# mjq11302010044/TATT

Measured on AMD Instinct MI355X. Metric: LR images/s (train fwd+bwd+clip+Adam) at 16x64->32x128, higher is better.
Workload: dtype fp32 (split-bf16 MFMA operands in conv3 / conv3-wgrad / conv9 / tokgemm / gru-wgrad / query-GRU recurrence and dW_hh / TP-layer backward)

## Files before the change

include/tatt_hip.h:

```cpp
#ifndef TATT_HIP_H
#define TATT_HIP_H

#ifdef __cplusplus
extern "C" {
#endif

typedef struct ihipStream_t* hipStream_t;


int tatt_gemm(const float* A, long sam, long sak, const float* A2, long sa2m, long sa2k, int K1,
              const float* B, long sbk, long sbn, const float* bias, float* C, long scm, long scn,
              int M, int N, int K, int Z, long bsA, long bsA2, long bsB, long bsC, long bsBias,
              float alpha, float beta, int act, int splitk, float* ws, float* rowsum, hipStream_t st);

int tatt_conv2d_fwd(const float* x, long xsn, long xsh, long xsw, long xsc, const float* wpacked,
                    const float* bias, float* y, long ldy, int Bn, int H, int W, int Cin, int Cout,
                    int KH, int KW, int act, float beta, int splitk, float* ws, hipStream_t st);

int tatt_conv2d_fwd_partials(const float* x, long xsn, long xsh, long xsw, long xsc, const float* wpacked, int Bn, int H,
                             int W, int Cin, int Cout, int KH, int KW, int splitk, float* ws, int* splits, hipStream_t st);

int tatt_conv2d_wgrad(const float* x, long xsn, long xsh, long xsw, long xsc, const float* dy,
                      long lddy, float* dw_oihw, int Bn, int H, int W, int Cin, int Cout, int KH,
                      int KW, float beta, int splitk, float* ws, hipStream_t st);
// ... 64 lines not shown
                         const float* beta, float* mean, float* rstd, float* running_mean, float* running_var, float* scale,
                         float* shift, hipStream_t st);
int tatt_bn_rstd(const float* var, float* rstd, int C, float eps, hipStream_t st);
int tatt_bn_apply(const float* X, long ldx, float* Y, long ldy, int M, int C, const float* mean,
                  const float* rstd, const float* gamma, const float* beta, int act, hipStream_t st);
int tatt_bn_bwd(const float* X, long ldx, const float* dY, long lddy, float* dX, long lddx, int M, int C,
                const float* mean, const float* rstd, const float* gamma, const float* beta, int act,
                int training, float* dgamma, float* dbeta, float* sums, double* ws, hipStream_t st);
int tatt_bn_bwd_groups(int M);
int tatt_bn_bwd_partials(const float* X, long ldx, const float* dY, long lddy, int M, int C, const float* mean,
                         const float* rstd, const float* gamma, const float* beta, int act, double* part, hipStream_t st);
int tatt_bn_bwd_finish(const double* part, int G, int C, int M, const float* mean, const float* rstd, const float* gamma,
                       float* dgamma, float* dbeta, float* coef, hipStream_t st);
int tatt_bn_bwd_affine(const float* X, const float* dU, float* dX, int M, int C, const float* coef, hipStream_t st);

int tatt_ln_fwd(const float* A, const float* Bres, float* Y, float* stats, int M, int C,
                const float* gamma, const float* beta, float eps, int mode, float pdrop,
                const unsigned long long* seed, unsigned site, hipStream_t st);
int tatt_ln_bwd(const float* A, const float* Bres, const float* dY, const float* stats, float* dX, float* dB, int M,
                int C, const float* gamma, float* dgamma, float* dbeta, float* part, double* ws, float eps, int mode,
                float pdrop, const unsigned long long* seed, unsigned site, hipStream_t st);


int tatt_prelu_fwd(const float* x, float* y, const float* alpha, long n, hipStream_t st);
int tatt_prelu_bwd(const float* x, const float* dy, float* dx, const float* alpha, long n, float* part,
                   hipStream_t st);
int tatt_act_fwd(const float* x, float* y, long n, int act, hipStream_t st);
int tatt_act_bwd(const float* ref, const float* dy, float* dx, long n, int act, int from_output,
                 hipStream_t st);
int tatt_axpby(const float* a, const float* b, float* y, float alpha, float beta, long n, hipStream_t st);
int tatt_add_n(const float* const* srcs, int n, float* y, long numel, hipStream_t st);
int tatt_add_rowbcast(const float* a, const float* b, float* y, long rows, int C, long period,
                      hipStream_t st);
int tatt_pixel_shuffle_fwd(const float* in, float* out, int B, int H, int W, int C, int act,
                           hipStream_t st);
int tatt_pixel_shuffle_bwd(const float* in, const float* dout, float* din, int B, int H, int W, int C,
                           int act, hipStream_t st);
int tatt_maxpool_fwd(const float* in, float* out, int B, int H, int W, int C, int kh, int kw, int sh, int sw,
                     int ph, int pw, hipStream_t st);
int tatt_maxpool_bwd(const float* in, const float* dout, float* din, int B, int H, int W, int C, int kh,
                     int kw, int sh, int sw, int ph, int pw, hipStream_t st);
int tatt_dropout(const float* x, float* y, long n, float p, const unsigned long long* seed, unsigned site,
                 hipStream_t st);
int tatt_bump_seed(unsigned long long* seed, unsigned long long* snap, hipStream_t st);
int tatt_stamp(unsigned long long* out, hipStream_t st);
int tatt_copy4d(const float* src, float* dst, int n0, int n1, int n2, int n3, long s0, long s1, long s2,
                long s3, long d0, long d1, long d2, long d3, float beta, hipStream_t st);


int tatt_l2norm(const float* g, long n, float* out, double* ws, hipStream_t st);
int tatt_adam_step(float* p, const float* g, float* m, float* v, long n, float lr, float b1, float b2,
                   float eps, const float* gnorm, float max_norm, float gscale, const long long* step,
                   hipStream_t st);


int tatt_gru32_fwd(const float* gi, const float* whh_f, const float* bhh_f, const float* whh_r,
                   const float* bhh_r, float* out, float* gates, int nseq, int T, int s_in, long stride_hi,
                   long stride_lo, long stride_t, hipStream_t st);
int tatt_gru32_bwd(const float* gates, const float* out, const float* dout, const float* whh_f,
                   const float* whh_r, float* dgi, float* dgh, float* hprev, int nseq, int T, int s_in,
                   long stride_hi, long stride_lo, long stride_t, hipStream_t st);

int tatt_gru32_fwd2(const float* gi, const float* whh_f, const float* bhh_f, const float* whh_r,
                    const float* bhh_r, float* out, float* gates, int nseq, int T, int s_in, long stride_hi,
                    long stride_lo, long stride_t, hipStream_t st);
int tatt_gru32_bwd2(const float* gates, const float* out, const float* dout, const float* whh_f,
                    const float* whh_r, float* dgi, float* dgh, float* hprev, float* frag, int nseq, int T, int s_in,
                    long stride_hi, long stride_lo, long stride_t, hipStream_t st);
int tatt_gru_wgrad_frag(const float* frag, const float* x, const float* xb, float* ws1, float* ws2, int nseq, int T,
                        int s_in, long stride_hi, long stride_lo, long stride_t, int G, hipStream_t st);
int tatt_gru_wgrad_frag_in(const float* frag, const float* x, const float* xb, float* ws1, float* ws2, int nseq, int T,
                           int s_in, long stride_hi, long stride_lo, long stride_t, int G, const float* in_mean,
                           const float* in_rstd, const float* in_gamma, const float* in_beta, const float* in_add,
                           hipStream_t st);

int tatt_qgru_bwd_fused(const float* dgh_cur0, const float* dgh_cur1, const float* whhT0, const float* whhT1,
                        const float* dhseq_next0, const float* dhseq_next1, const float* gsave_next0,
                        const float* gsave_next1, const float* hprev_next0, const float* hprev_next1,
                        float* dhcarry0, float* dhcarry1, float* dgi_acc0, float* dgi_acc1, float* dgh_next0,
                        float* dgh_next1, int Wb, int HID, hipStream_t st);

int tatt_gru_compose(const float* wih_f, const float* wih_r, const float* bih_f, const float* bih_r,
                     const float* Wc, const float* bc, float* Wp, float* bp, int K, hipStream_t st);
int tatt_gru_compose_batch(const float* const* ptrs, const int* Ks, int n, hipStream_t st);
int tatt_gru_tail(const float* dWp, const float* dbp, const float* Wc, const float* bc, const float* wih_f,
                  const float* wih_r, float* dwih_f, float* dwih_r, float* dWc, float* dbc, int K,
                  const float* dWhh, float* dwhh_f, float* dwhh_r, hipStream_t st);

int tatt_gru_tail_c(const float* dWp, const float* dbp, const float* Wc, const float* bc, const float* wih_f,
                    const float* wih_r, float* dwih_f, float* dwih_r, float* dWc, float* dbc, int K,
                    const float* dWhh_c, float* dwhh_f, float* dwhh_r, hipStream_t st);

int tatt_qgru_fwd_step(const float* gi0, const float* gi1, const float* whh0, const float* whh1,
                       const float* bhh0, const float* bhh1, const float* hprev0, const float* hprev1,
                       float* hnew0, float* hnew1, float* gsave0, float* gsave1, int Wb, int HID,
                       hipStream_t st);
int tatt_qgru_bwd_gates(const float* dhseq0, const float* dhseq1, const float* gsave0, const float* gsave1,
                        const float* hprev0, const float* hprev1, float* dhcarry0, float* dhcarry1,
                        float* dgi_acc0, float* dgi_acc1, float* dgh0, float* dgh1, int Wb, int HID, int first,
                        hipStream_t st);
int tatt_qgru_bwd_mm(const float* dgh0, const float* dgh1, const float* whhT0, const float* whhT1,
                     float* dhcarry0, float* dhcarry1, int Wb, int HID, hipStream_t st);

int tatt_qgru_bwd_chain(float* dgh0, float* dgh1, const float* whhT0, const float* whhT1, const float* dhseq0,
                        const float* dhseq1, const float* gsave0, const float* gsave1, const float* hbuf0,
                        const float* hbuf1, float* dhcarry0, float* dhcarry1, float* dgi_acc0, float* dgi_acc1,
// ... 270 lines not shown
```

tatt_amd/csrc/elementwise.hip:

```cpp
#include "common.h"

#define EW_GRID(total) dim3(cdiv((total), 256)), dim3(256)

__global__ void prelu_fwd_kernel(const float* __restrict__ x, float* __restrict__ y, const float* __restrict__ a,
                                 long n) {
    long i = (long)blockIdx.x * blockDim.x + threadIdx.x;
    if (i >= n) return;
    float v = x[i];
    y[i] = v >= 0.f ? v : a[0] * v;
}
TATT_API int tatt_prelu_fwd(const float* x, float* y, const float* alpha, long n, hipStream_t st) {
    hipLaunchKernelGGL(prelu_fwd_kernel, EW_GRID(n), 0, st, x, y, alpha, n);
    return LAUNCH_CHECK();
}
__global__ void prelu_bwd_kernel(const float* __restrict__ x, const float* __restrict__ dy, float* __restrict__ dx,
                                 const float* __restrict__ a, long n, float* __restrict__ part) {
    __shared__ double sh[4];
    long i = (long)blockIdx.x * blockDim.x + threadIdx.x;
    double s = 0.0;
    if (i < n) {
        float v = x[i], g = dy[i];
        dx[i] = v >= 0.f ? g : a[0] * g;
        if (v < 0.f) s = (double)g * (double)v;
    }
// ... 319 lines not shown
    s = wave_sum_d(s);
    if ((threadIdx.x & 63) == 0) sh[threadIdx.x >> 6] = s;
    __syncthreads();
    if (threadIdx.x == 0) out[0] = (float)sqrt((sh[0] + sh[1]) + (sh[2] + sh[3]));
}
TATT_API int tatt_l2norm(const float* g, long n, float* out, double* ws, hipStream_t st) {
    int G = (int)((n + 255) / 256);
    if (G > 1024) G = 1024;
    if (G < 1) G = 1;
    hipLaunchKernelGGL(sumsq_stage1, dim3(G), dim3(256), 0, st, g, n, ws);
    hipLaunchKernelGGL(sumsq_stage2, dim3(1), dim3(256), 0, st, ws, G, out);
    return LAUNCH_CHECK();
}
__device__ __forceinline__ void adam_one(float& p, float g, float& m, float& v, float coef, float b1, float b2, float a1, float rs2,
                                         float eps) {
    const float gi = g * coef;
    const float mi = b1 * m + (1.f - b1) * gi;
    const float vi = b2 * v + (1.f - b2) * gi * gi;
    m = mi; v = vi;
    p -= a1 * mi / (sqrtf(vi) * rs2 + eps);
}
__global__ void adam_kernel(float* __restrict__ p, const float* __restrict__ g, float* __restrict__ m,
                            float* __restrict__ v, long n, float lr, float b1, float b2, float eps,
                            const float* __restrict__ gnorm, float max_norm, float gscale,
                            const long long* __restrict__ step) {
    const long i = (long)blockIdx.x * blockDim.x + threadIdx.x;
    const long n4 = n >> 2;
    if (i > n4) return;
    const double t = (double)step[0];
    const float bc1 = (float)(1.0 - pow((double)b1, t)), bc2 = (float)(1.0 - pow((double)b2, t));
    float coef = gscale;
    if (max_norm > 0.f) { float c = max_norm / (gnorm[0] * gscale + 1e-6f); coef *= c < 1.f ? c : 1.f; }
    const float a1 = lr / bc1, rs2 = 1.f / sqrtf(bc2);
    if (i < n4) {
        float4 pp = ((float4*)p)[i], mm = ((float4*)m)[i], vv = ((float4*)v)[i];
        const float4 gg = ((const float4*)g)[i];
        adam_one(pp.x, gg.x, mm.x, vv.x, coef, b1, b2, a1, rs2, eps);
        adam_one(pp.y, gg.y, mm.y, vv.y, coef, b1, b2, a1, rs2, eps);
        adam_one(pp.z, gg.z, mm.z, vv.z, coef, b1, b2, a1, rs2, eps);
        adam_one(pp.w, gg.w, mm.w, vv.w, coef, b1, b2, a1, rs2, eps);
        ((float4*)p)[i] = pp; ((float4*)m)[i] = mm; ((float4*)v)[i] = vv;
    } else {
        for (long k = n4 << 2; k < n; ++k) adam_one(p[k], g[k], m[k], v[k], coef, b1, b2, a1, rs2, eps);
    }
}
TATT_API int tatt_adam_step(float* p, const float* g, float* m, float* v, long n, float lr, float b1, float b2,
                            float eps, const float* gnorm, float max_norm, float gscale, const long long* step,
                            hipStream_t st) {
    if (((uintptr_t)p | (uintptr_t)g | (uintptr_t)m | (uintptr_t)v) & 15) return 1001;
    hipLaunchKernelGGL(adam_kernel, EW_GRID((n >> 2) + 1), 0, st, p, g, m, v, n, lr, b1, b2, eps, gnorm, max_norm, gscale, step);
    return LAUNCH_CHECK();
}

#include <mutex>
static std::mutex g_sticky_mu;
static unsigned* g_sticky[64] = {};
unsigned* tatt_sticky_ptr() {
    int dev = 0;
    if (hipGetDevice(&dev) != hipSuccess || dev < 0 || dev >= 64) return nullptr;
    std::lock_guard<std::mutex> lk(g_sticky_mu);
    return g_sticky[dev];
}
TATT_API int tatt_set_sticky(unsigned* word) {
    int dev = 0;
    if (hipGetDevice(&dev) != hipSuccess || dev < 0 || dev >= 64) return 1;
    std::lock_guard<std::mutex> lk(g_sticky_mu);
    g_sticky[dev] = word;
    return 0;
}
__global__ void sync_guard_kernel(const unsigned* word) {
    if (__hip_atomic_load(word, __ATOMIC_RELAXED, __HIP_MEMORY_SCOPE_AGENT) != 0u) __builtin_trap();
}
TATT_API int tatt_sync_guard(hipStream_t st) {
    unsigned* w = tatt_sticky_ptr();
    if (!w) return 0;
    hipLaunchKernelGGL(sync_guard_kernel, dim3(1), dim3(1), 0, st, w);
    return LAUNCH_CHECK();
}

__global__ __launch_bounds__(512) void cu_holder_kernel(long ticks, unsigned* sink, int lds_words) {
    extern __shared__ unsigned hold_lds[];
    for (int i = threadIdx.x; i < lds_words; i += 512) hold_lds[i] = i;
    __syncthreads();
    const long t0 = wall_clock64();
    unsigned acc = 0;
    while (wall_clock64() - t0 < ticks) {
        acc += lds_words ? hold_lds[(threadIdx.x + acc) % lds_words] : 1u;
        __builtin_amdgcn_s_sleep(8);
    }
    if (acc == 0xffffffffu && sink) sink[0] = acc;
}
TATT_API int tatt_cu_holder(int groups, long ticks, int lds_bytes, unsigned* sink, hipStream_t st) {
    if (groups < 1 || groups > 1024 || ticks < 0 || ticks > 100000000L || lds_bytes < 0 || lds_bytes > 65536) return 1;
    hipLaunchKernelGGL(cu_holder_kernel, dim3(groups), dim3(512), lds_bytes, st, ticks, sink, lds_bytes / 4);
    return LAUNCH_CHECK();
}

#define GG_MAX 112
struct GGEntry { const float* src; long off; int n; int block0; };
struct GGTable { GGEntry e[GG_MAX]; float* dst; int n; };
__global__ __launch_bounds__(256) void gather_grads_kernel(GGTable t) {
    int k = 0;
    while (k + 1 < t.n && (int)blockIdx.x >= t.e[k + 1].block0) ++k;
    const GGEntry& e = t.e[k];
    const long i = ((long)((int)blockIdx.x - e.block0) * 256 + threadIdx.x) * 4;
    if (i >= e.n) return;
// ... 42 lines not shown
```

tatt_amd/csrc/gemm.hip:

```cpp
#include "common.h"
#include <mutex>
#include <unordered_map>
#include <stdlib.h>

#define BM 64
#define BN 64
#define KC 16
#define LDT 65

struct GemmP {
    const float* A; const float* A2; const float* B; const float* bias; float* C;
    int M, N, K, K1;
    long sam, sak, sa2m, sa2k, sbk, sbn, scm, scn;
    long bsA, bsA2, bsB, bsC, bsBias;
    float alpha, beta;
    int act;
    int splitk, chunks_per_split;
    float* partial;
    float* rowsum;
    int H, W, Cin, KH, KW, pad, HW, Wshift, HWshift, Cshift;
    long xsn, xsh, xsw, xsc;
};

__device__ __forceinline__ void decode_pixel(const GemmP& p, int pix, int& n, int& h, int& w) {
// ... 882 lines not shown
    if (mode >= 12) {
        if (idx < TOEPLITZ9_WORDS) out[idx] = toeplitz9_sb(w, idx, mode);
        return;
    }
    if (mode >= 10) {
        if (idx < Cout * Cin * 9) out[idx] = repack_sb(w, idx, Cout, Cin, mode);
        return;
    }
    if (mode >= 8) {
        if (idx < TOEPLITZ9_WORDS) out[idx] = toeplitz9(w, idx, mode);
        return;
    }
    int total = Cout * Cin * KH * KW;
    if (idx >= total) return;
    int T = KH * KW;
    if (mode == 0) {
        int co = idx % Cout; int r = idx / Cout; int ci = r % Cin; int tap = r / Cin;
        out[idx] = w[((long)co * Cin + ci) * T + tap];
    } else if (mode == 1) {
        int ci = idx % Cin; int r = idx / Cin; int co = r % Cout; int tap = r / Cout;
        out[idx] = w[((long)co * Cin + ci) * T + (T - 1 - tap)];
    } else if (mode == 2) {
        int ci = idx % Cin; int r = idx / Cin; int co = r % Cout; int tap = r / Cout;
        out[idx] = w[((long)co * Cin + ci) * T + tap];
    } else if (mode == 3) {
        int co = idx % Cout; int r = idx / Cout; int ci = r % Cin; int tap = r / Cin;
        out[idx] = w[((long)co * Cin + ci) * T + (T - 1 - tap)];
    } else {
        const int u = idx & 3, lane = (idx >> 2) & 63;
        const int q6 = (idx >> 8) % 36, blk = idx / (36 * 256);
        const int tap6 = q6 >> 2, g6 = q6 & 3;
        const int o6 = blk * 16 + (lane & 15), i6 = 16 * g6 + 4 * (lane >> 4) + u;
        if (mode == 6) out[idx] = w[((long)o6 * Cin + i6) * T + tap6];
        else out[idx] = w[((long)i6 * Cin + o6) * T + (T - 1 - tap6)];
    }
}
TATT_API int tatt_repack_words(int Cout, int Cin, int KH, int KW, int mode) {
    if (mode == 4 || mode == 5 || mode < 0 || mode > 15) return -1;
    return (int)repack_total(Cout, Cin, KH, KW, mode);
}
TATT_API int tatt_repack_conv_weight(const float* w_oihw, float* out, int Cout, int Cin, int KH, int KW,
                                     int mode, hipStream_t st) {
    const bool fwd9 = mode == 8 || mode == 12, dgrad9 = mode == 9 || mode == 13;
    if ((fwd9 || dgrad9) && !(KH == 9 && KW == 9 && ((fwd9 && Cout == 4 && Cin == 64) || (dgrad9 && Cout == 64 && Cin == 4)))) return 1;
    if ((mode == 10 || mode == 11 || mode == 14 || mode == 15) && !(KH == 3 && KW == 3 && Cout % 64 == 0 && Cin % 64 == 0)) return 1;
    if (mode == 4 || mode == 5 || mode < 0 || mode > 15) return 1;
    long total = repack_total(Cout, Cin, KH, KW, mode);
    hipLaunchKernelGGL(repack_weight_kernel, dim3(cdiv(total, 256)), dim3(256), 0, st, w_oihw, out, Cout, Cin,
                       KH, KW, mode);
    return LAUNCH_CHECK();
}

#define REPACK_MAX 96
struct RepackEntry { const float* w; float* out; int Cout, Cin, KH, KW, mode, block0; };
struct RepackTable { RepackEntry e[REPACK_MAX]; int n; };
__global__ void repack_batch_kernel(RepackTable t) {
    int k = 0;
    while (k + 1 < t.n && (int)blockIdx.x >= t.e[k + 1].block0) ++k;
    const RepackEntry& e = t.e[k];
    const int idx = ((int)blockIdx.x - e.block0) * blockDim.x + threadIdx.x;
    if (e.mode >= 14) {
        if (idx < e.Cout * e.Cin * 9) e.out[idx] = repack_sb32(e.w, idx, e.Cout, e.Cin, e.mode);
        return;
    }
    if (e.mode >= 12) {
        if (idx < TOEPLITZ9_WORDS) e.out[idx] = toeplitz9_sb(e.w, idx, e.mode);
        return;
    }
    if (e.mode >= 10) {
        if (idx < e.Cout * e.Cin * 9) e.out[idx] = repack_sb(e.w, idx, e.Cout, e.Cin, e.mode);
        return;
    }
    if (e.mode >= 8) {
        if (idx < TOEPLITZ9_WORDS) e.out[idx] = toeplitz9(e.w, idx, e.mode);
        return;
    }
    const int total = e.Cout * e.Cin * e.KH * e.KW;
    if (idx >= total) return;
    const int T = e.KH * e.KW, Cout = e.Cout, Cin = e.Cin;
    const float* w = e.w;
    float v;
    if (e.mode == 0) { int co = idx % Cout; int r = idx / Cout; int ci = r % Cin; int tap = r / Cin; v = w[((long)co * Cin + ci) * T + tap]; }
    else if (e.mode == 1) { int ci = idx % Cin; int r = idx / Cin; int co = r % Cout; int tap = r / Cout; v = w[((long)co * Cin + ci) * T + (T - 1 - tap)]; }
    else if (e.mode == 2) { int ci = idx % Cin; int r = idx / Cin; int co = r % Cout; int tap = r / Cout; v = w[((long)co * Cin + ci) * T + tap]; }
    else if (e.mode == 3) { int co = idx % Cout; int r = idx / Cout; int ci = r % Cin; int tap = r / Cin; v = w[((long)co * Cin + ci) * T + (T - 1 - tap)]; }
    else {
        const int u = idx & 3, lane = (idx >> 2) & 63;
        const int q6 = (idx >> 8) % 36, blk = idx / (36 * 256);
        const int tap6 = q6 >> 2, g6 = q6 & 3;
        const int o6 = blk * 16 + (lane & 15), i6 = 16 * g6 + 4 * (lane >> 4) + u;
        v = e.mode == 6 ? w[((long)o6 * Cin + i6) * T + tap6] : w[((long)i6 * Cin + o6) * T + (T - 1 - tap6)];
    }
    e.out[idx] = v;
}
TATT_API int tatt_repack_conv_weight_batch(const float* const* ws, float* const* outs, const int* dims, int n, hipStream_t st) {
    if (n <= 0) return 0;
    for (int base = 0; base < n; base += REPACK_MAX) {
        RepackTable t;
        t.n = n - base < REPACK_MAX ? n - base : REPACK_MAX;
        int blocks = 0;
        for (int k = 0; k < t.n; ++k) {
            const int* d = dims + (long)(base + k) * 5;
            t.e[k] = {ws[base + k], outs[base + k], d[0], d[1], d[2], d[3], d[4], blocks};
            blocks += cdiv(repack_total(d[0], d[1], d[2], d[3], d[4]), 256);
        }
        hipLaunchKernelGGL(repack_batch_kernel, dim3(blocks), dim3(256), 0, st, t);
    }
    return LAUNCH_CHECK();
}

TATT_API int tatt_splitk_reduce(const float* partial, float* C, int M, int N, int S, int remap_cin, int remap_taps,
                                float beta, float* vec, int vec_len, hipStream_t st) {
    ReduceArgs a = {partial, C, nullptr, vec, (long)N, 1L, 0L, 0L, M, N, S, 1, 1.f, beta, (int)ACT_NONE, remap_cin, remap_taps, 0,
                    vec ? vec_len : 0};
    return reduce_submit(a, st);
}
```

tatt_amd/train.py:

```python
from __future__ import annotations

import os
from typing import Optional

import torch

from . import functional as Fh
from . import ops
from .dp import FlatParams, GradCuts, broadcast_model, rank_dropout_seed


def image_loss(sr, hr, weights=(1.0, 1e-4)):
    return Fh.ImageLossFn.apply(sr, hr, float(weights[0]), float(weights[1]), None)


def image_loss_mean(sr, hr, weights=(1.0, 1e-4), scale=100.0):
    return Fh.ImageLossFn.apply(sr, hr, float(weights[0]), float(weights[1]), float(scale))


def semantic_loss(pred, gt):
    return Fh.SemanticLossFn.apply(pred, gt.detach())


_CTC_ROW_OFFS = {}
# ... 205 lines not shown
STUDENT_FORK = False
TEACHER_AHEAD = True


class TssimRecipe:

    def __init__(self, rotate_train=5.0, seed=0, off_range=0.2):
        import numpy as np
        self.rotate_train, self.off_range = float(rotate_train), off_range
        self.rng = np.random.RandomState(seed)
        self.theta_pos = self.theta_neg = None
        self.last = None

    def draw(self, B):
        import math
        arcs = torch.tensor((self.rng.rand(B) * self.rotate_train * 2 - self.rotate_train) / 180.0 * math.pi).float()
        offs = torch.tensor(self.rng.rand(B)).float()
        return arcs, offs

    def new_step(self, x, arcs=None, offs=None):
        from .losses import rotation_theta
        B, _, H, W = x.shape
        if arcs is None:
            arcs, offs = self.draw(B)
        self.last = (arcs, offs)
        pos, neg = rotation_theta(arcs, offs, H, W, self.off_range), rotation_theta(-arcs, offs, H, W, self.off_range)
        if self.theta_pos is None:
            self.theta_pos, self.theta_neg = pos.to(x.device), neg.to(x.device)
        else:
            self.theta_pos.copy_(pos)
            self.theta_neg.copy_(neg)

    def loss(self, model, x, tp, hr):
        from .losses import TRI_SSIM
        rot = Fh.AffineSampleFn.apply
        with torch.no_grad():
            x_rot, hr_rot = rot(x, self.theta_pos), rot(hr, self.theta_pos)
            x_ret = rot(x_rot, self.theta_neg)
        fwd = (lambda im: model(im, tp)) if tp is not None else model
        fwd_ret = (lambda im: model(im, reuse_prior=True)) if (tp is None and hasattr(model, "tpg")) else fwd
        if hasattr(model, "begin_teacher"):
            model.begin_teacher(hr_rot)
        out = fwd(x_rot)
        sr = out[0] if isinstance(out, tuple) else out
        extra = model.extra_loss(hr_rot) if hasattr(model, "extra_loss") else None
        out = fwd_ret(x_ret)
        sr_ret = out[0] if isinstance(out, tuple) else out
        l_img = image_loss_mean(sr, hr_rot, scale=100.0)
        l_tssim = (1.0 - TRI_SSIM()(rot(sr_ret, self.theta_pos), sr, hr_rot)) * 10.0
        loss = l_img + l_tssim
        return loss if extra is None else loss + extra


class HipStepKernels:

    def l2norm(self, g, out, ws):
        ops.call("tatt_l2norm", ops.P(g), g.numel(), ops.P(out), ops.P(ws), ops.stream())

    def adam(self, p, g, m, v, lr, b1, b2, eps, gnorm, max_norm, gscale, step):
        ops.call("tatt_adam_step", ops.P(p), ops.P(g), ops.P(m), ops.P(v), p.numel(), lr, b1, b2, eps, ops.P(gnorm), max_norm,
                 gscale, ops.P(step), ops.stream())

    def inc(self, counter):
        ops.inc_i64(counter)

    def guard(self):
        ops.call("tatt_sync_guard", ops.stream())

    def after_update(self, device):
        ops.PACKED.refresh(device)


def _default_loss(sr, hr):
    return image_loss_mean(sr, hr, scale=100.0)


class Trainer:

    def __init__(self, model, lr=1e-3, betas=(0.5, 0.999), eps=1e-8, clip=0.25, use_graph=False, warmup_eager=2,
                 process_group=None, broadcast_init=True, defer_param_grads=True, side_stream=True, kernels=None, loss_fn=None,
                 dropout_seed=None, recipe=None):
        self.model = model
        self.lr, self.betas, self.eps, self.clip = lr, betas, eps, clip
        self.pg = process_group
        self.dp = process_group is not None
        self.world = torch.distributed.get_world_size(process_group) if self.dp else 1
        self.rank = torch.distributed.get_rank(process_group) if self.dp else 0
        self.kernels = kernels if kernels is not None else HipStepKernels()
        self.loss_fn = loss_fn if loss_fn is not None else _default_loss
        self.recipe = recipe
        self.profile_collectives = False
        self._coll_events = []
        self._group_events = []
        dev = next(model.parameters()).device
        self.dev = dev
        self.cuda = dev.type == "cuda"
        self.defer = bool(defer_param_grads)
        self.two_lanes = self.defer and bool(side_stream) and self.cuda
        staged = (self.dp or self.defer) and hasattr(model, "grad_buckets") and hasattr(model, "set_grad_cuts")
        buckets = None
        if hasattr(model, "grad_buckets"):
            import inspect
            takes_dp = "dp" in inspect.signature(model.grad_buckets).parameters
            buckets = model.grad_buckets(dp=self.dp) if takes_dp else model.grad_buckets()
        if buckets is not None and not staged:
            buckets = [("all", [p for _, ps in buckets for p in ps])]
        self.flat = FlatParams(model, buckets)
        self.stages = self.flat.bucket_names
        self._due = {id(p): k for k, (_, ps) in enumerate(buckets or []) for p in ps}
        self._immediate = frozenset(id(p) for p in model.immediate_grad_params()) if hasattr(model, "immediate_grad_params") else frozenset()
        self.cuts = GradCuts() if staged and len(self.stages) > 1 else None
        self.params = self.flat.params
        self.n = self.flat.n
        self.flat_p, self.flat_g = self.flat.p, self.flat.g
        self.flat_m = torch.zeros(self.n, device=dev)
        self.flat_v = torch.zeros(self.n, device=dev)
        groups = model.clip_groups(clip) if hasattr(model, "clip_groups") else [(self.params, clip)]
        self.groups = [self.flat.span(ps) + (float(c),) for ps, c in groups]
        assert sorted(self.groups)[0][0] == 0 and sum(e - s for s, e, _ in self.groups) == self.n
        if self.dp and broadcast_init:
# ... 50 lines not shown
                    extra = self.model.extra_loss(hr) if hasattr(self.model, "extra_loss") else None
                    if extra is not None:
                        loss = loss + extra
                if self._one is None or self._one.device != loss.device or self._one.dtype != loss.dtype:
                    self._one = torch.ones_like(loss)
                loss.backward(self._one)
                self.last_loss = loss.detach()
            else:
                self.cuts.run(self.stages[k])
        finally:
            Fh.SIDE.enabled = False
            Fh.SIDE.side_stream = None
            Fh.FWD_FORK.enabled = Fh.FWD_FORK_B.enabled = False
            if k == 0 and self.cuts is not None:
                self.model.set_grad_cuts(None)
        if k == len(self.stages) - 1 and hasattr(self.model, "block"):
            self.model.block = None

    def _side_lane(self, k):
        Fh.SIDE.flush(None if k == len(self.stages) - 1 else k)
        self.flat.gather_grads(k)

    def _pass(self, k, x=None, tp=None, hr=None):
        nst = len(self.stages)
        main = torch.cuda.current_stream(self.dev) if self.cuda else None
        merge_last = self._merge_last
        if merge_last and k == nst:
            return
        name = self.stages[k] if k < nst and isinstance(self.stages[k], str) else str(k)
        Fh.stamp("pass %s: start" % name)
        if k >= 1:
            if self.two_lanes:
                self.side.wait_stream(main)
                with torch.cuda.stream(self.side):
                    self._side_lane(k - 1)
                    Fh.stamp("pass %s: side lane done" % name)
            else:
                self._side_lane(k - 1)
        if k < nst:
            self._main_lane(k, x, tp, hr)
            Fh.stamp("pass %s: main lane done" % name)
        joined = False
        if merge_last and k == nst - 1:
            Fh.SIDE.flush(None)
            if k >= 1 and self.two_lanes:
                main.wait_stream(self.side)
                joined = True
            self.flat.gather_grads(k)
            Fh.stamp("pass %s: merged side work done" % name)
        if k >= 1 and self.two_lanes and not joined:
            main.wait_stream(self.side)

    def _optim(self):
        if self.cuda and hasattr(self.kernels, "guard"):
            self.kernels.guard()
        if hasattr(self.kernels, "inc"):
            self.kernels.inc(self.step_count)
        else:
            self.step_count += 1
        b1, b2 = self.betas
        for (s, e, max_norm), gn in zip(self.groups, self.gnorms):
            if max_norm > 0.0:
                self.kernels.l2norm(self.flat_g[s:e], gn, self.norm_ws)
            self.kernels.adam(self.flat_p[s:e], self.flat_g[s:e], self.flat_m[s:e], self.flat_v[s:e], self.lr, b1, b2, self.eps,
                              gn, max_norm, 1.0 / self.world, self.step_count)
        if hasattr(self.kernels, "after_update"):
            self.kernels.after_update(self.dev)

    def _reduce(self, lo, hi, after_pass):
        if self.dp and hi >= lo:
            self.reduce_log.append((after_pass, lo, hi))
            s, e = self.flat.ranges[lo][0], self.flat.ranges[hi][1]
            self._works.append(torch.distributed.all_reduce(self.flat.g[s:e], op=torch.distributed.ReduceOp.SUM, group=self.pg,
                                                            async_op=True))

    def _buckets_done_by(self, k):
        nst = len(self.stages)
        return nst - 1 if (self._merge_last and k >= nst - 1) else min(k - 1, nst - 1)

    def _wait_reduces(self):
        prof = self.profile_collectives and self.cuda
        for i, w in enumerate(self._works):
            if prof:
                e0, e1 = torch.cuda.Event(enable_timing=True), torch.cuda.Event(enable_timing=True)
                e0.record()
                w.wait()
                e1.record()
                self._coll_events.append((i, e0, e1))
                del self._coll_events[:-self.PROFILE_KEEP]
            else:
                w.wait()
        self._works = []

    PROFILE_KEEP = 256

    def collective_report(self):
        if not self.dp:
            return None
        rep = {"backend": torch.distributed.get_backend(self.pg), "world_size": torch.distributed.get_world_size(self.pg),
               "per_step": [{"after_pass": ap, "buckets": [self.flat.bucket_names[k] for k in range(lo, hi + 1)],
                             "bytes": 4 * (self.flat.ranges[hi][1] - self.flat.ranges[lo][0])} for ap, lo, hi in self.reduce_log]}
        if self._coll_events:
            torch.cuda.synchronize(self.dev)
            n = max(i for i, _, _ in self._coll_events) + 1
            tot, cnt = [0.0] * n, [0] * n
            for i, e0, e1 in self._coll_events:
# ... 98 lines not shown
```

Measured before the change: 11480.

## Fuse optimizer tail into partial-norm and Adam kernels; tile weight repack through LDS

The optimizer tail now runs one kernel per group that computes sum-of-squares partials, with the sticky guard check and step increment folded into the first group's launch. A second kernel reduces those partials, applies clipping and performs the Adam update over a grid capped by CU count. This removes the separate guard, increment and l2norm-finalize launches. Separately, the post-update conv weight repack now stages tiles in shared memory and emits vectorized, coalesced writes instead of doing a strided gather per element, at the cost of more complex tiling logic.

```diff
diff --git a/include/tatt_hip.h b/include/tatt_hip.h
--- a/include/tatt_hip.h
+++ b/include/tatt_hip.h
@@ -140,6 +140,11 @@
 int tatt_adam_step(float* p, const float* g, float* m, float* v, long n, float lr, float b1, float b2,
                    float eps, const float* gnorm, float max_norm, float gscale, const long long* step,
                    hipStream_t st);
+int tatt_l2norm_partials(const float* g, long n, double* ws, int guard, long long* step, hipStream_t st);
+int tatt_adam_step_partials(float* p, const float* g, float* m, float* v, long n, float lr, float b1, float b2,
+                            float eps, const double* parts, int nparts, float* gnorm_out, float max_norm, float gscale,
+                            const long long* step, hipStream_t st);
+int tatt_adam_groups_per_cu(int per_cu);
 
 
 int tatt_gru32_fwd(const float* gi, const float* whh_f, const float* bhh_f, const float* whh_r,
diff --git a/tatt_amd/csrc/elementwise.hip b/tatt_amd/csrc/elementwise.hip
--- a/tatt_amd/csrc/elementwise.hip
+++ b/tatt_amd/csrc/elementwise.hip
@@ -395,6 +395,104 @@
     return LAUNCH_CHECK();
 }
 
+__global__ __launch_bounds__(256) void sumsq_partials_kernel(const float* __restrict__ g, long n, double* __restrict__ part,
+                                                             const unsigned* sticky, long long* step) {
+    __shared__ double sh[4];
+    if (sticky && __hip_atomic_load(sticky, __ATOMIC_RELAXED, __HIP_MEMORY_SCOPE_AGENT) != 0u) __builtin_trap();
+    if (step && blockIdx.x == 0 && threadIdx.x == 0) step[0] += 1;
+    const long stride = (long)gridDim.x * 256;
+    double s = 0.0;
+    for (long i = (long)blockIdx.x * 256 + threadIdx.x; i < n; i += 8 * stride) {
+        float a[8];
+#pragma unroll
+        for (int j = 0; j < 8; ++j) { const long k = i + j * stride; a[j] = g[k < n ? k : n - 1]; }
+#pragma unroll
+        for (int j = 0; j < 8; ++j) {
+            double v = i + j * stride < n ? (double)a[j] : 0.0;
+            s += v * v;
+        }
+    }
+    s = wave_sum_d(s);
+    if ((threadIdx.x & 63) == 0) sh[threadIdx.x >> 6] = s;
+    __syncthreads();
+    if (threadIdx.x == 0) part[blockIdx.x] = (sh[0] + sh[1]) + (sh[2] + sh[3]);
+}
+static inline int l2norm_groups(long n) {
+    long G = (n + 255) / 256;
+    return G > 1024 ? 1024 : (G < 1 ? 1 : (int)G);
+}
+TATT_API int tatt_l2norm_partials(const float* g, long n, double* ws, int guard, long long* step, hipStream_t st) {
+    hipLaunchKernelGGL(sumsq_partials_kernel, dim3(l2norm_groups(n)), dim3(256), 0, st, g, n, ws, guard ? tatt_sticky_ptr() : nullptr,
+                       step);
+    return LAUNCH_CHECK();
+}
+__global__ __launch_bounds__(256) void adam_partials_kernel(float* __restrict__ p, const float* __restrict__ g, float* __restrict__ m,
+                                                            float* __restrict__ v, long n, float lr, float b1, float b2, float eps,
+                                                            const double* __restrict__ parts, int nparts, float* __restrict__ gnorm_out,
+                                                            float max_norm, float gscale, const long long* __restrict__ step) {
+    __shared__ double sh[4];
+    __shared__ float sc[3];
+    if (max_norm > 0.f) {
+        double s = 0.0;
+        for (int i = threadIdx.x; i < nparts; i += 256) s += parts[i];
+        s = wave_sum_d(s);
+        if ((threadIdx.x & 63) == 0) sh[threadIdx.x >> 6] = s;
+    }
+    __syncthreads();
+    if (threadIdx.x == 0) {
+        const double t = (double)step[0];
+        const float bc1 = (float)(1.0 - pow((double)b1, t)), bc2 = (float)(1.0 - pow((double)b2, t));
+        float coef = gscale;
+        if (max_norm > 0.f) {
+            const float gnorm = (float)sqrt((sh[0] + sh[1]) + (sh[2] + sh[3]));
+            if (blockIdx.x == 0) gnorm_out[0] = gnorm;
+            float c = max_norm / (gnorm * gscale + 1e-6f);
+            coef *= c < 1.f ? c : 1.f;
+        }
+        sc[0] = coef; sc[1] = lr / bc1; sc[2] = 1.f / sqrtf(bc2);
+    }
+    __syncthreads();
+    const float coef = sc[0], a1 = sc[1], rs2 = sc[2];
+    const long n4 = n >> 2, stride = (long)gridDim.x * 256;
+    for (long i = (long)blockIdx.x * 256 + threadIdx.x; i <= n4; i += stride) {
+        if (i < n4) {
+            float4 pp = ((float4*)p)[i], mm = ((float4*)m)[i], vv = ((float4*)v)[i];
+            const float4 gg = ((const float4*)g)[i];
+            adam_one(pp.x, gg.x, mm.x, vv.x, coef, b1, b2, a1, rs2, eps);
+            adam_one(pp.y, gg.y, mm.y, vv.y, coef, b1, b2, a1, rs2, eps);
+            adam_one(pp.z, gg.z, mm.z, vv.z, coef, b1, b2, a1, rs2, eps);
+            adam_one(pp.w, gg.w, mm.w, vv.w, coef, b1, b2, a1, rs2, eps);
+            ((float4*)p)[i] = pp; ((float4*)m)[i] = mm; ((float4*)v)[i] = vv;
+        } else {
+            for (long k = n4 << 2; k < n; ++k) adam_one(p[k], g[k], m[k], v[k], coef, b1, b2, a1, rs2, eps);
+        }
+    }
+}
+static int g_adam_groups_per_cu = 8;
+TATT_API int tatt_adam_groups_per_cu(int per_cu) {
+    if (per_cu < 1 || per_cu > 64) return 1;
+    g_adam_groups_per_cu = per_cu;
+    return 0;
+}
+TATT_API int tatt_adam_step_partials(float* p, const float* g, float* m, float* v, long n, float lr, float b1, float b2,
+                                     float eps, const double* parts, int nparts, float* gnorm_out, float max_norm, float gscale,
+                                     const long long* step, hipStream_t st) {
+    if (((uintptr_t)p | (uintptr_t)g | (uintptr_t)m | (uintptr_t)v) & 15) return 1001;
+    if (max_norm > 0.f && (nparts < 1 || nparts > 1024 || !parts || !gnorm_out)) return 1;
+    static int cus[64] = {};
+    int dev = 0;
+    if (hipGetDevice(&dev) != hipSuccess || dev < 0 || dev >= 64) return 1;
+    if (!cus[dev]) {
+        int c = 0;
+        if (hipDeviceGetAttribute(&c, hipDeviceAttributeMultiprocessorCount, dev) != hipSuccess || c < 1) return 1;
+        cus[dev] = c;
+    }
+    const long need = ((n >> 2) + 256) / 256, cap = (long)cus[dev] * g_adam_groups_per_cu;
+    hipLaunchKernelGGL(adam_partials_kernel, dim3((unsigned)(need < cap ? need : cap)), dim3(256), 0, st, p, g, m, v, n, lr, b1, b2, eps,
+                       parts, nparts, gnorm_out, max_norm, gscale, step);
+    return LAUNCH_CHECK();
+}
+
 #include <mutex>
 static std::mutex g_sticky_mu;
 static unsigned* g_sticky[64] = {};
diff --git a/tatt_amd/csrc/gemm.hip b/tatt_amd/csrc/gemm.hip
--- a/tatt_amd/csrc/gemm.hip
+++ b/tatt_amd/csrc/gemm.hip
@@ -958,13 +958,188 @@
 }
 
 #define REPACK_MAX 96
-struct RepackEntry { const float* w; float* out; int Cout, Cin, KH, KW, mode, block0; };
+#define RP_TILE 4608
+#define RP_LDS 5120
+struct RepackEntry { const float* w; float* out; int Cout, Cin, block0; short T; unsigned char mode, flags; short nco, nci; };
 struct RepackTable { RepackEntry e[REPACK_MAX]; int n; };
-__global__ void repack_batch_kernel(RepackTable t) {
-    int k = 0;
-    while (k + 1 < t.n && (int)blockIdx.x >= t.e[k + 1].block0) ++k;
-    const RepackEntry& e = t.e[k];
-    const int idx = ((int)blockIdx.x - e.block0) * blockDim.x + threadIdx.x;
+struct RpTile { int co0, nco, ci0, nci, t0, nt, pitch; long ob; };
+#define RP_TILED 1
+#define RP_VEC 2
+static int repack_plan(RepackEntry& e, int KH, int KW) {
+    const int Cout = e.Cout, Cin = e.Cin, T = e.T, mode = e.mode;
+    const bool al = ((uintptr_t)e.out & 15) == 0, k3 = KH == 3 && KW == 3, k9 = KH == 9 && KW == 9;
+    e.flags = 0; e.nco = e.nci = 0;
+    auto tiles = [&](int n) { e.flags |= RP_TILED | RP_VEC; return n; };
+    switch (mode) {
+    case 0: case 3: case 1: case 2: {
+        if (Cout < 1 || Cin < 1 || T < 1 || T > RP_TILE || KH * KW > 32767) break;
+        int nco, nci;
+        if (mode == 0 || mode == 3) {
+            nco = Cout < 32 ? Cout : 32;
+            if (nco * T > RP_TILE) nco = RP_TILE / T;
+            nci = RP_TILE / (nco * T);
+            if (nci > Cin) nci = Cin;
+            if (al && Cout % 4 == 0 && nco % 4 == 0) e.flags |= RP_VEC;
+        } else {
+            nci = Cin < 32 ? Cin : 32;
+            if (nci * T > RP_TILE) nci = RP_TILE / T;
+            nco = RP_TILE / (nci * T);
+            if (nco > Cout) nco = Cout;
+            if (nco > 256) nco = 256;
+            if (al && Cin % 4 == 0 && nci % 4 == 0) e.flags |= RP_VEC;
+        }
+        e.nco = (short)nco; e.nci = (short)nci; e.flags |= RP_TILED;
+        return cdiv(Cout, nco) * cdiv(Cin, nci);
+    }
+    case 6: if (al && k3 && Cin == 64 && Cout % 16 == 0 && Cout > 0) return tiles(Cout / 16 * 4); break;
+    case 7: if (al && k3 && Cout == 64 && Cin % 16 == 0 && Cin > 0) return tiles(Cin / 16 * 4); break;
+    case 8: case 12: if (al && k9 && Cout == 4 && Cin == 64) return tiles(36); break;
+    case 9: case 13: if (al && k9 && Cout == 64 && Cin == 4) return tiles(36); break;
+    case 10: case 11: if (al && k3 && Cout % 64 == 0 && Cin % 64 == 0 && Cout > 0 && Cin > 0) return tiles(Cout / 16 * (Cin / 16) / 2); break;
+    case 14: case 15: if (al && k3 && Cout % 64 == 0 && Cin % 64 == 0 && Cout > 0 && Cin > 0) return tiles(Cout / 16 * (Cin / 16) / 2); break;
+    }
+    return cdiv(repack_total(Cout, Cin, KH, KW, mode), 256);
+}
+__device__ __forceinline__ RpTile rp_tile(const RepackEntry& e, int ti) {
+    RpTile t;
+    const int mode = e.mode, dg = mode & 1;
+    t.t0 = 0; t.nt = e.T; t.ob = 0;
+    if (mode < 4) {
+        const int tci = (e.Cin + e.nci - 1) / e.nci, a = ti / tci, b = ti - a * tci;
+        t.co0 = a * e.nco; t.ci0 = b * e.nci;
+        t.nco = e.Cout - t.co0 < e.nco ? e.Cout - t.co0 : e.nco;
+        t.nci = e.Cin - t.ci0 < e.nci ? e.Cin - t.ci0 : e.nci;
+    } else if (mode < 8) {
+        const int g = ti & 3, blk = ti >> 2;
+        t.co0 = dg ? 16 * g : 16 * blk; t.ci0 = dg ? 16 * blk : 16 * g; t.nco = t.nci = 16;
+        t.ob = (long)(blk * 36 + g) * 256;
+    } else if (mode < 10 || mode == 12 || mode == 13) {
+        const int c = ti & 3, ky = ti >> 2;
+        t.co0 = dg ? 16 * c : 0; t.nco = dg ? 16 : 4; t.ci0 = dg ? 0 : 16 * c; t.nci = dg ? 4 : 16;
+        t.t0 = dg ? (8 - ky) * 9 : ky * 9; t.nt = 9;
+        t.ob = (long)ti * 3072;
+    } else if (mode < 12) {
+        const int half = ti & 1, r = ti >> 1, nblk = (dg ? e.Cin : e.Cout) / 16, chunk = r / nblk, blk = r - chunk * nblk;
+        const int o0 = 16 * blk, i0 = 64 * chunk + 32 * half;
+        t.co0 = dg ? i0 : o0; t.nco = dg ? 32 : 16; t.ci0 = dg ? o0 : i0; t.nci = dg ? 16 : 32;
+        t.ob = (long)r * 9216 + half * 512;
+    } else {
+        const int ks = ti & 3, r = ti >> 2, nblk = (dg ? e.Cin : e.Cout) / 32, chunk = r / nblk, blk = r - chunk * nblk;
+        const int o0 = 32 * blk, i0 = 64 * chunk + 16 * ks;
+        t.co0 = dg ? i0 : o0; t.nco = dg ? 16 : 32; t.ci0 = dg ? o0 : i0; t.nci = dg ? 32 : 16;
+        t.ob = (long)r * 18432 + ks * 512;
+    }
+    t.pitch = (t.nci * t.nt) | 1;
+    return t;
+}
+#define RP_INFLIGHT 18
+template <bool FULL>
+__device__ __forceinline__ void rp_stage(const RepackEntry& e, const RpTile t, float* lds, int tid) {
+    const int rowlen = t.nci * t.nt, T = e.T, nt = t.nt, wave = tid >> 6, lane = tid & 63, per_row = (rowlen + 63) >> 6;
+    const int chunks = ((t.nco - wave + 3) >> 2) * per_row;
+    const long rstride = (long)e.Cin * T;
+    const float* __restrict__ w = e.w + ((long)t.co0 * e.Cin + t.ci0) * T + t.t0;
+    int k = 0, c = 0;
+    for (int m0 = 0; m0 < chunks; m0 += RP_INFLIGHT) {
+        float a[RP_INFLIGHT];
+        const int k0 = k, c0 = c;
+#pragma unroll
+        for (int j = 0; j < RP_INFLIGHT; ++j) {
+            const int r = 64 * c + lane, rc = r < rowlen ? r : rowlen - 1, col = FULL ? 0 : rc / nt;
+            a[j] = w[(wave + 4 * k) * rstride + (FULL ? (long)rc : (long)col * T + (rc - col * nt))];
+            if (m0 + j + 1 < chunks && ++c == per_row) { c = 0; ++k; }
+        }
+        k = k0; c = c0;
+#pragma unroll
+        for (int j = 0; j < RP_INFLIGHT; ++j) {
+            const int r = 64 * c + lane;
+            if (m0 + j < chunks && r < rowlen) lds[(wave + 4 * k) * t.pitch + r] = a[j];
+            if (m0 + j + 1 < chunks && ++c == per_row) { c = 0; ++k; }
+        }
+    }
+}
+__device__ __forceinline__ float rp_split(float a, float b, int hl) {
+    const rp_f32x2 v = (rp_f32x2){a, b};
+    const rp_bf16x2 hi = __builtin_convertvector(v, rp_bf16x2);
+    const rp_bf16x2 lo = __builtin_convertvector(v - __builtin_convertvector(hi, rp_f32x2), rp_bf16x2);
+    return __builtin_bit_cast(float, hl ? lo : hi);
+}
+__device__ __forceinline__ void rp_emit(const RepackEntry& e, const RpTile t, const float* lds, int tid) {
+    const int mode = e.mode, dg = mode & 1, T = e.T, P = t.pitch, nt = t.nt, co0 = t.co0, ci0 = t.ci0, nco = t.nco, nci = t.nci;
+    float* __restrict__ out = e.out;
+#define RP_S(row, col, tap) lds[(row) * P + (col) * nt + (tap)]
+    if (mode < 4) {
+        const bool rows_fast = mode == 0 || mode == 3, flip = mode == 1 || mode == 3;
+        const int nfast = rows_fast ? nco : nci, nslow = rows_fast ? nci : nco, fs = rows_fast ? P : nt, ss = rows_fast ? nt : P;
+        const long Nfast = rows_fast ? e.Cout : e.Cin, Nslow = rows_fast ? e.Cin : e.Cout;
+        const int f0 = rows_fast ? co0 : ci0, s0 = rows_fast ? ci0 : co0;
+        const int per = (e.flags & RP_VEC) ? nfast >> 2 : nfast, items = T * nslow * per;
+        for (int q = tid; q < items; q += 256) {
+            const int r = q / per, f = q - r * per, tap = r / nslow, sl = r - tap * nslow;
+            const float* s = lds + sl * ss + (flip ? T - 1 - tap : tap);
+            float* o = out + ((long)tap * Nslow + s0 + sl) * Nfast + f0;
+            if (e.flags & RP_VEC) {
+                s += 4 * f * fs;
+                *reinterpret_cast<f32x4*>(o + 4 * f) = (f32x4){s[0], s[fs], s[2 * fs], s[3 * fs]};
+            } else o[f] = s[f * fs];
+        }
+        return;
+    }
+    if (mode < 8) {
+        for (int q = tid; q < 9 * 64; q += 256) {
+            const int tap = q >> 6, lane = q & 63, ol = lane & 15, il = 4 * (lane >> 4);
+            f32x4 v;
+#pragma unroll
+            for (int u = 0; u < 4; ++u) v[u] = dg ? RP_S(il + u, ol, 8 - tap) : RP_S(ol, il + u, tap);
+            *reinterpret_cast<f32x4*>(out + (t.ob + tap * 1024 + lane * 4)) = v;
+        }
+        return;
+    }
+    if (mode < 10) {
+        for (int q = tid; q < 12 * 64; q += 256) {
+            const int lane = q & 63, r = q >> 6, kh = r / 6, f = r - 6 * kh, cqi = f / 3, d = f - 3 * cqi;
+            const int cl = 4 * (kh + 2 * cqi) + (lane >> 4), nn = lane & 15, j = nn >> 2, o = nn & 3;
+            f32x4 v;
+#pragma unroll
+            for (int u = 0; u < 4; ++u) {
+                const int kx = 4 * d + u - j, kc = kx < 0 ? 0 : (kx > 8 ? 8 : kx);
+                const float x = dg ? RP_S(cl, o, 8 - kc) : RP_S(o, cl, kc);
+                v[u] = kx == kc ? x : 0.f;
+            }
+            *reinterpret_cast<f32x4*>(out + (t.ob + q * 4)) = v;
+        }
+        return;
+    }
+    if (mode == 12 || mode == 13) {
+        for (int q = tid; q < 12 * 64; q += 256) {
+            const int lane = q & 63, hl = (q >> 6) & 1, pair = q >> 7, nn = lane & 15, kq = lane >> 4, j = nn >> 2, o = nn & 3;
+            const int kx = 2 * pair + (kq >> 1) - j, kc = kx < 0 ? 0 : (kx > 8 ? 8 : kx), cl = 8 * (kq & 1);
+            f32x4 v;
+#pragma unroll
+            for (int e2 = 0; e2 < 4; ++e2) {
+                const float a = dg ? RP_S(cl + 2 * e2, o, 8 - kc) : RP_S(o, cl + 2 * e2, kc);
+                const float b = dg ? RP_S(cl + 2 * e2 + 1, o, 8 - kc) : RP_S(o, cl + 2 * e2 + 1, kc);
+                v[e2] = kx == kc ? rp_split(a, b, hl) : rp_split(0.f, 0.f, hl);
+            }
+            *reinterpret_cast<f32x4*>(out + (t.ob + q * 4)) = v;
+        }
+        return;
+    }
+    const int sh = mode < 12 ? 4 : 5, om = (1 << sh) - 1, run = mode < 12 ? 1024 : 2048;
+    for (int q = tid; q < 9 * 128; q += 256) {
+        const int tap = q >> 7, hl = (q >> 6) & 1, lane = q & 63, ol = lane & om, il = 8 * (lane >> sh);
+        f32x4 v;
+#pragma unroll
+        for (int e2 = 0; e2 < 4; ++e2) {
+            const float a = dg ? RP_S(il + 2 * e2, ol, 8 - tap) : RP_S(ol, il + 2 * e2, tap);
+            const float b = dg ? RP_S(il + 2 * e2 + 1, ol, 8 - tap) : RP_S(ol, il + 2 * e2 + 1, tap);
+            v[e2] = rp_split(a, b, hl);
+        }
+        *reinterpret_cast<f32x4*>(out + (t.ob + (long)tap * run + hl * 256 + lane * 4)) = v;
+    }
+#undef RP_S
+}
+__device__ __forceinline__ void rp_gather(const RepackEntry& e, int idx) {
     if (e.mode >= 14) {
         if (idx < e.Cout * e.Cin * 9) e.out[idx] = repack_sb32(e.w, idx, e.Cout, e.Cin, e.mode);
         return;
@@ -981,9 +1156,8 @@
         if (idx < TOEPLITZ9_WORDS) e.out[idx] = toeplitz9(e.w, idx, e.mode);
         return;
     }
-    const int total = e.Cout * e.Cin * e.KH * e.KW;
-    if (idx >= total) return;
-    const int T = e.KH * e.KW, Cout = e.Cout, Cin = e.Cin;
+    const int T = e.T, Cout = e.Cout, Cin = e.Cin;
+    if (idx >= Cout * Cin * T) return;
     const float* w = e.w;
     float v;
     if (e.mode == 0) { int co = idx % Cout; int r = idx / Cout; int ci = r % Cin; int tap = r / Cin; v = w[((long)co * Cin + ci) * T + tap]; }
@@ -999,6 +1173,29 @@
     }
     e.out[idx] = v;
 }
+__device__ __forceinline__ void repack_batch_block(const RepackTable& t, float* lds, int bid, int tid, int phase) {
+    int lo = 0, hi = t.n - 1;
+    while (lo < hi) {
+        const int mid = (lo + hi + 1) >> 1;
+        if (bid >= t.e[mid].block0) lo = mid; else hi = mid - 1;
+    }
+    const RepackEntry& e = t.e[lo];
+    const int ti = bid - e.block0;
+    if (!(e.flags & RP_TILED)) {
+        if (phase == 0) rp_gather(e, ti * 256 + tid);
+        return;
+    }
+    const RpTile tl = rp_tile(e, ti);
+    if (phase == 1) rp_emit(e, tl, lds, tid);
+    else if (tl.nt == e.T) rp_stage<true>(e, tl, lds, tid);
+    else rp_stage<false>(e, tl, lds, tid);
+}
+__global__ __launch_bounds__(256) void repack_batch_kernel(RepackTable t) {
+    __shared__ float lds[RP_LDS];
+    repack_batch_block(t, lds, (int)blockIdx.x, (int)threadIdx.x, 0);
+    __syncthreads();
+    repack_batch_block(t, lds, (int)blockIdx.x, (int)threadIdx.x, 1);
+}
 TATT_API int tatt_repack_conv_weight_batch(const float* const* ws, float* const* outs, const int* dims, int n, hipStream_t st) {
     if (n <= 0) return 0;
     for (int base = 0; base < n; base += REPACK_MAX) {
@@ -1007,10 +1204,11 @@
         int blocks = 0;
         for (int k = 0; k < t.n; ++k) {
             const int* d = dims + (long)(base + k) * 5;
-            t.e[k] = {ws[base + k], outs[base + k], d[0], d[1], d[2], d[3], d[4], blocks};
-            blocks += cdiv(repack_total(d[0], d[1], d[2], d[3], d[4]), 256);
-        }
-        hipLaunchKernelGGL(repack_batch_kernel, dim3(blocks), dim3(256), 0, st, t);
+            if (d[4] < 0 || d[4] > 15 || d[2] < 0 || d[3] < 0 || (long)d[2] * d[3] > 32767) return 1;
+            t.e[k] = {ws[base + k], outs[base + k], d[0], d[1], blocks, (short)(d[2] * d[3]), (unsigned char)d[4], 0, 0, 0};
+            blocks += repack_plan(t.e[k], d[2], d[3]);
+        }
+        if (blocks) hipLaunchKernelGGL(repack_batch_kernel, dim3(blocks), dim3(256), 0, st, t);
     }
     return LAUNCH_CHECK();
 }
diff --git a/tatt_amd/train.py b/tatt_amd/train.py
--- a/tatt_amd/train.py
+++ b/tatt_amd/train.py
@@ -281,6 +281,9 @@
         return loss if extra is None else loss + extra
 
 
+FUSED_TAIL = True
+
+
 class HipStepKernels:
 
     def l2norm(self, g, out, ws):
@@ -295,6 +298,24 @@
 
     def guard(self):
         ops.call("tatt_sync_guard", ops.stream())
+
+    def chain(self, groups, p, g, m, v, gnorms, lr, b1, b2, eps, gscale, step, ws):
+        lead = next((k for k, (_, _, c) in enumerate(groups) if c > 0.0), None)
+        if lead is None:
+            self.guard()
+            self.inc(step)
+        elif lead > 0:
+            groups, gnorms = list(groups), list(gnorms)
+            groups.insert(0, groups.pop(lead))
+            gnorms.insert(0, gnorms.pop(lead))
+        for k, ((s, e, max_norm), gn) in enumerate(zip(groups, gnorms)):
+            n, nparts = e - s, 0
+            if max_norm > 0.0:
+                nparts = min(1024, max(1, (n + 255) // 256))
+                ops.call("tatt_l2norm_partials", ops.P(g[s:e]), n, ops.P(ws), int(k == 0), ops.P(step) if k == 0 else None,
+                         ops.stream())
+            ops.call("tatt_adam_step_partials", ops.P(p[s:e]), ops.P(g[s:e]), ops.P(m[s:e]), ops.P(v[s:e]), n, lr, b1, b2, eps,
+                     ops.P(ws), nparts, ops.P(gn), max_norm, gscale, ops.P(step), ops.stream())
 
     def after_update(self, device):
         ops.PACKED.refresh(device)
@@ -451,6 +472,13 @@
             main.wait_stream(self.side)
 
     def _optim(self):
+        if FUSED_TAIL and self.cuda and hasattr(self.kernels, "chain"):
+            b1, b2 = self.betas
+            self.kernels.chain(self.groups, self.flat_p, self.flat_g, self.flat_m, self.flat_v, self.gnorms, self.lr, b1, b2,
+                               self.eps, 1.0 / self.world, self.step_count, self.norm_ws)
+            if hasattr(self.kernels, "after_update"):
+                self.kernels.after_update(self.dev)
+            return
         if self.cuda and hasattr(self.kernels, "guard"):
             self.kernels.guard()
         if hasattr(self.kernels, "inc"):
```

Measured after the change: 11550, median of 6. No clear change (+0.6%).
